# kcleal/pywfa

Hardware: AMD Instinct MI355X
Metric: pairwise alignments/sec (higher is better)
Workload: dtype int16x2 offsets (reads <= 512 bp), int32 results; 1 GPU; C2: 10000000 x 150bp pairs/GPU, 2% error, gap-affine 0/4/6/2, end-to-end, scope=score, 2-bit reads resident in HBM; pairs_per_gpu=10000000, read_length=150, parallelism=pairs sharded over 1 GPU(s), no collective

## Files before the change

pywfa_amd/csrc/host_core.hpp:

```cpp
#pragma once
#include <hip/hip_runtime.h>
#include <stdint.h>
#include <stdio.h>
#include <stdlib.h>
#include <string.h>
#include <limits.h>
#include <sched.h>
#include <string>
#include <map>
#include <unordered_map>
#include <vector>
#include <algorithm>
#include <thread>
#include <memory>
#include <atomic>

#include "wfa_hip.h"
#include "wfa_common.hpp"
#include "wfa_band.hpp"

namespace wfa { struct WfaPieceDesc; }

#pragma GCC visibility push(hidden)

extern thread_local std::string g_error;

#define WFA_COUNTER_WORDS 256
#define WFA_KNOBS(F)                                                                                              \
  F(ARENA_KB) F(BAND_DEBUG) F(BAND_SLIM) F(BAND_LDS_MAX) F(BAND_NO_WIN) F(BAND_SPLIT_MIN) F(NO_TINY_INLINE) F(BILEVEL) F(BILEVEL_WIDE_LEVELS) F(BILEVEL_PER_CU) F(BILEVEL_I32) F(BILEVEL_QCAP) F(BILEVEL_LEVELS) F(BILEVEL_LDS) F(BILEVEL_NO_1024) F(BILEVEL_HUGE_MIN) F(BILEVEL_LDS_W) F(BILEVEL_NO_SEQL) F(LANE_DYN) F(LANE_DYN_WAVES) F(BAND_LEFTOVER_WAVES_PER_CU) F(BAND_NCH) F(BAND_NO_LDS) F(BAND_NO_SPLIT) F(BAND_PB) F(PIPE_TAIL) F(LEN16) F(MAILBOX) F(MAILBOX_IDLE_US) F(TILE32)     \
  F(BAND_RECORDS) F(BAND_SPLIT_ROUNDS) F(BAND_WAVES_PER_CU) F(NO_BAND) F(NO_FAST) F(NO_SEGFULL) F(SEGFULL_PAIRS)     \
  F(SEGFULL_STAGES) F(STAGE_TIMING) F(LANE_HEUR32) F(THREADS) F(TINY_BATCH) F(WAVES_PER_CU) F(FAST_WAVES_PER_CU) F(TIMING)          \
  F(LANE_FULL) F(LANE_FULL_SPLIT) F(LANE_HEUR) F(SEG_HEUR) F(LANE_LDS_PAD_KB) F(LANE_MIN_PAIRS) F(PIPE_CHUNK) F(PIPE_THREADS) F(PACK_THREADS) F(NO_TINY_BAND) F(NO_TINY_POLL) F(UP_STREAMS) F(NO_DUAL) F(NO_WIDE) F(WIDE_ADAPT) F(WIDE_GROWS) F(WIDE_LDS_KB) F(WIDE_THREADS) F(TILE) F(TILE_T) F(TILE_WT) F(TILE_THREADS) F(TILE_PER_CU) F(NO_PIPE) F(HOST_PACK) F(GENERAL_PB) F(LANE_WAVES_PER_CU) F(LANE_REFILL_MIN) F(LANE_DEBUG) F(NO_TINY) F(PILOT_PCT) F(WIDE_ADAPT_LDS) F(LANE_NARROW_WAVES) F(PILOT_NARROW_PCT) F(CROSS_BAND) F(CROSS_TOPK_CHUNK) F(REDUCE_TIMING)
enum WfaKnob {
#define WFA_KNOB_ENUM(n) K_##n,
  WFA_KNOBS(WFA_KNOB_ENUM)
#undef WFA_KNOB_ENUM
  K_COUNT
};
struct WfaKnobs {
  int value[K_COUNT];
  bool set[K_COUNT];
  std::string fast_stages;
  void load() {
    static const char* const names[K_COUNT] = {
#define WFA_KNOB_NAME(n) "WFA_HIP_" #n,
        WFA_KNOBS(WFA_KNOB_NAME)
#undef WFA_KNOB_NAME
    };
    for (int i = 0; i < K_COUNT; ++i) {
      const char* v = getenv(names[i]);
      set[i] = v && *v;
      value[i] = set[i] ? atoi(v) : 0;
    }
    const char* fs = getenv("WFA_HIP_FAST_STAGES");
    fast_stages = (fs && *fs) ? fs : "";
  }
};

struct wfa_hip_aligner {
  int numa_state = 0;
  int numa_node = -1;
  cpu_set_t numa_cpus;
  int numa_mode = 0;
  cpu_set_t proc_cpus;
  bool proc_cpus_valid = false;
// ... 174 lines not shown
```

pywfa_amd/csrc/wfa_hip.hip:

```cpp
#include <hip/hip_runtime.h>
#include <stdint.h>
#include <stdio.h>
#include <stdlib.h>
#include <string.h>
#include <limits.h>
#include <string>
#include <map>
#include <unordered_map>
#include <vector>
#include <algorithm>
#include <chrono>
#include <thread>
#include <memory>
#include <atomic>
#include <mutex>
#include <functional>
#include <ctype.h>
#include <pthread.h>
#include <sched.h>
#include <unistd.h>
#include <sys/syscall.h>

#include "host_core.hpp"
#include "wfa_pack.hpp"
// ... 1107 lines not shown
  }
  al->err = "pilot launch failed";
  return WFA_HIP_EDEVICE;
}

static int pilot_first_width(wfa_hip_aligner* al, wfa_hip_batch* b, hipStream_t stream) {
  const unsigned rtc_failures = wfa::rtc_failure_count();
  const bool full = (b->cfg.scope == WFA_SCOPE_FULL);
  if (b->stage_pick != 0 || b->n_packed < 65536u) return WFA_HIP_OK;
  if (!wfa::seg_supported(b->dcfg, b->ncomp, false) || b->max_len > WFA_FAST_MAX_LEN || knob(al, K_NO_FAST, 0) != 0) return WFA_HIP_OK;
  if (full ? (knob(al, K_NO_SEGFULL, 0) != 0 || al->knobs.set[K_SEGFULL_STAGES]) : !al->knobs.fast_stages.empty()) return WFA_HIP_OK;
  const uint32_t np = 8192u, stride = b->n_packed / np;
  uint32_t* plist = b->d_fb_list2[0];
  uint32_t* psample = b->d_fb_list2[1];
  uint32_t* pcount = b->d_counters + 4;
  hipLaunchKernelGGL(wfa_pilot_sample_kernel, dim3((np + 255u) / 256u), dim3(256), 0, stream, b->d_list_packed, stride, np, psample);
  HIP_TRY(al, hipGetLastError());
  b->stage_pick = 128;
  for (int w = 16; w <= 64; w *= 2) {
    HIP_TRY(al, hipMemsetAsync(pcount, 0, sizeof(uint32_t), stream));
    if (wfa::launch_seg(b->dcfg, al->cu_count, knob(al, K_FAST_WAVES_PER_CU, 256), stream, b->d_words, b->d_meta, psample, nullptr, np, b->d_score, b->d_status,
                        plist, pcount, w == 16 ? 2 : (w == 32 ? 4 : 5)) != 0) return pilot_launch_failed(al, b, rtc_failures);
    uint32_t handed = 0;
    HIP_TRY(al, hipMemcpyAsync(&handed, pcount, sizeof(uint32_t), hipMemcpyDeviceToHost, stream));
    HIP_TRY(al, hipStreamSynchronize(stream));
    const uint32_t pct = (w == 16) ? (uint32_t)knob(al, K_PILOT_PCT, full ? 15 : 8) : 40u;
    if (knob(al, K_STAGE_TIMING, 0)) fprintf(stderr, "[wfa_hip] pilot: %d diagonals hand on %u of %u\n", w, handed, np);
    if (handed * 100u <= np * pct) { b->stage_pick = w; break; }
  }
  int X, OE, E;
  if (!full && b->stage_pick == 16 && wfa::seg_shape(b->dcfg, &X, &OE, &E) != WFA_SHAPE_RTC) {
    HIP_TRY(al, hipMemsetAsync(pcount, 0, sizeof(uint32_t), stream));
    if (wfa::launch_lane(wfa::seg_shape(b->dcfg, &X, &OE, &E), wfa::gcd_int(wfa::gcd_int(b->dcfg.x, b->dcfg.o1 + b->dcfg.e1), b->dcfg.e1), al->cu_count,
                         knob(al, K_LANE_WAVES_PER_CU, 48), knob(al, K_LANE_REFILL_MIN, 8), b->max_len, stream, b->d_words, b->d_meta, psample, nullptr, np,
                         b->d_score, b->d_status, plist, pcount, nullptr, 0, X, OE, E, 0, nullptr, 0, 4) != 0) return pilot_launch_failed(al, b, rtc_failures);
    uint32_t handed = 0;
    HIP_TRY(al, hipMemcpyAsync(&handed, pcount, sizeof(uint32_t), hipMemcpyDeviceToHost, stream));
    HIP_TRY(al, hipStreamSynchronize(stream));
    const uint32_t pct = (uint32_t)knob(al, K_PILOT_NARROW_PCT, 20);
    if (knob(al, K_STAGE_TIMING, 0)) fprintf(stderr, "[wfa_hip] pilot: 8 diagonals (lane form) hand on %u of %u\n", handed, np);
    b->narrow_pick = (handed * 100u <= np * pct) ? 1 : 2;
    b->narrow_permille = (int)((uint64_t)handed * 1000u / np);
  }
  HIP_TRY(al, hipMemsetAsync(pcount, 0, sizeof(uint32_t), stream));
  return WFA_HIP_OK;
}

static int pilot_band(wfa_hip_aligner* al, wfa_hip_batch* b, hipStream_t stream) {
  const unsigned rtc_failures = wfa::rtc_failure_count();
  if (b->band_pick != 0 || b->n_packed < 32768u) return WFA_HIP_OK;
  const bool two = b->ncomp == 5;
  if (b->dcfg.heuristic != WFA_HEUR_NONE || (b->ncomp != 3 && !two) || (two ? (b->max_len <= 100 || b->max_len > 2000) : (b->max_len <= 300 || b->max_len > 1200))) return WFA_HIP_OK;
  if (!wfa::band_supported(b->dcfg, b->ncomp) || knob(al, K_NO_BAND, 0) != 0 || knob(al, K_BAND_NCH, 0) != 0) return WFA_HIP_OK;
  const uint32_t np = 4096u, stride = b->n_packed / np;
  uint32_t* plist = b->d_fb_list2[0];
  uint32_t* psample = b->d_fb_list2[1];
  uint32_t* pcount = b->d_counters + 4;
  hipLaunchKernelGGL(wfa_pilot_sample_kernel, dim3((np + 255u) / 256u), dim3(256), 0, stream, b->d_list_packed, stride, np, psample);
  HIP_TRY(al, hipGetLastError());
  HIP_TRY(al, hipMemsetAsync(pcount, 0, sizeof(uint32_t), stream));
  wfa::BandArgs ba;
  memset(&ba, 0, sizeof(ba));
  ba.words = b->d_words; ba.meta = b->d_meta; ba.worklist = psample; ba.nwork = np;
  ba.score = b->d_score; ba.status = b->d_status; ba.fb_list = plist; ba.fb_count = pcount;
  fill_band_penalties(ba, b->dcfg, two);
  fill_heuristic(ba, b->dcfg);
  ba.xdrop = b->dcfg.xdrop; ba.scope = b->dcfg.scope;
// ... 946 lines not shown
  const char* stages_env = al->knobs.fast_stages.empty() ? nullptr : al->knobs.fast_stages.c_str();
  const char* stages = stages_env ? stages_env : "189";
  if (!stages_env && b->stage_pick != 0 && c.in_count == nullptr) {
    stages = (b->stage_pick == 16) ? (b->narrow_pick == 1 ? "0189" : "189") : (b->stage_pick == 32) ? "89" : "9";
  }
  int variants[6] = {-1, -1, -1, -1, -1, -1};
  int nv = 0;
  for (const char* c = stages; *c && nv < 6; ++c) {
    const int v = *c - '0';
    if (v < 0 || v > 9) continue;
    if (v <= 1) {
      if (p.shape == WFA_SHAPE_RTC && (v == 0 || !p.lane_shape_fits)) continue;
    }
    variants[nv++] = v;
  }
  if (nv == 0) variants[nv++] = 6;
  int lane_passes = 0;
  for (int pass = 0; pass < nv; ++pass) {
    uint32_t* out_list = c.out_list(b);
    uint32_t* out_count = c.next_count(b);
    StageTimer timer(al, stream);
    int lrc;
    if (variants[pass] <= 1) {
      const bool narrow = variants[pass] == 0;
      const int lane_k = lane_passes++;
      uint32_t lane_dyn = (c.in_n >= 65536u && lane_k < 2) ? (uint32_t)std::max(0, knob(al, K_LANE_DYN, 192)) : 0u;
      const int dyn_waves = narrow ? knob(al, K_LANE_NARROW_WAVES, 24) : knob(al, K_LANE_DYN_WAVES, 16);
      if (lane_dyn && c.in_count != nullptr) {
        const int64_t expect = (b->narrow_permille >= 0 && variants[0] == 0) ? (int64_t)c.in_n * b->narrow_permille / 1000 : 0;
        const int64_t per_wave = expect / std::max<int64_t>(1, (int64_t)al->cu_count * dyn_waves * 2);
        lane_dyn = (uint32_t)std::max<int64_t>(64, std::min<int64_t>(lane_dyn, per_wave));
      }
      lrc = wfa::launch_lane(p.shape, affine_gcd(b->dcfg), al->cu_count,
                             lane_dyn ? dyn_waves : knob(al, K_LANE_WAVES_PER_CU, 48), knob(al, K_LANE_REFILL_MIN, 8), b->max_len, stream, b->d_words, b->d_meta,
                             c.in_list, c.in_count, c.in_n, b->d_score, b->d_status, out_list, out_count,
                             (knob(al, K_LANE_DEBUG, 0) && al->ws) ? al->ws : nullptr, knob(al, K_LANE_LDS_PAD_KB, 0), p.sh_x, p.sh_oe, p.sh_e, knob(al, K_LANE_MIN_PAIRS, 0),
                             b->d_counters + (lane_k == 0 ? CNT_LANE_DYN0 : CNT_LANE_DYN1), lane_dyn, narrow ? 4 : 8);
      if (knob(al, K_LANE_DEBUG, 0) && al->ws) {
        unsigned long long c[10] = {0, 0, 0, 0, 0, 0, 0, 0, 0, 0};
        hipStreamSynchronize(stream); hipMemcpy(c, al->ws, sizeof(c), hipMemcpyDeviceToHost); hipMemset(al->ws, 0, sizeof(c));
        fprintf(stderr, "[wfa_hip] lane kernel: %llu wave-steps, %llu refills, %llu parked runs, %llu parked rounds, %llu probe blocks, %llu second-run rounds, "
                        "%llu hand-over blocks, %llu second runs, %llu entries, %llu entry rounds\n", c[0], c[1], c[2], c[3], c[4], c[5], c[6], c[7], c[8], c[9]);
      }
    } else {
      lrc = wfa::launch_seg(b->dcfg, al->cu_count, knob(al, K_FAST_WAVES_PER_CU, 256), stream, b->d_words, b->d_meta, c.in_list, c.in_count,
                            c.in_n, b->d_score, b->d_status, out_list, out_count, variants[pass]);
    }
    if (lrc != 0) { al->err = "fast kernel launch failed"; return WFA_HIP_EDEVICE; }
    if (timer.on) {
      uint32_t handed = 0;
      const float ms = timer.stop(out_count, &handed);
      fprintf(stderr, "[wfa_hip] stage %d (variant %d): %.3f ms, handed on %u pairs\n", pass, variants[pass], ms, handed);
    }
    c.advance(b, out_list, out_count);
  }
  return WFA_HIP_OK;
}

static int run_laneh_stage(wfa_hip_aligner* al, wfa_hip_batch* b, hipStream_t stream, const CascadePlan& p, Chain& c) {
  uint32_t* out_list = c.out_list(b);
  uint32_t* out_count = c.next_count(b);
  wfa::FastArgs fa;
  memset(&fa, 0, sizeof(fa));
  fa.words = b->d_words; fa.meta = b->d_meta; fa.worklist = c.in_list; fa.nwork_dev = c.in_count; fa.nwork = c.in_n;
  fa.score = b->d_score; fa.status = b->d_status; fa.fb_list = out_list; fa.fb_count = out_count;
  fa.g = affine_gcd(b->dcfg);
  fill_ends_free(fa, b->dcfg, true);
// ... 1071 lines not shown
```

pywfa_amd/csrc/wfa_lane.hpp:

```cpp
#pragma once
#include "wfa_rtc_compat.hpp"
#include "wfa_common.hpp"
#include "wfa_hip.h"
#ifndef __HIPCC_RTC__
#include "wfa_rtc.hpp"
#endif

namespace wfa {

typedef short lane_s2 __attribute__((ext_vector_type(2)));
typedef unsigned short lane_u2 __attribute__((ext_vector_type(2)));

#define WFA_LANE_NULL16 (-16384)
#define WFA_LANE_NULL2 0xC000C000u
#ifndef WFA_LANE_DEBUG_COUNTERS
#define WFA_LANE_DEBUG_COUNTERS 0
#endif
#ifndef WFA_LANE_REGION_MARKS
#define WFA_LANE_REGION_MARKS 0
#endif
#if WFA_LANE_REGION_MARKS
#define WFA_LANE_MARK(name) asm volatile("; WFA_MARK " name ::: "memory")
#else
#define WFA_LANE_MARK(name)
// ... 36 lines not shown
#endif
}

#ifndef WFA_LANE_WAVES_PER_EU
#define WFA_LANE_WAVES_PER_EU 0
#endif
#if WFA_LANE_WAVES_PER_EU > 0
#define WFA_LANE_OCCUPANCY __attribute__((amdgpu_waves_per_eu(WFA_LANE_WAVES_PER_EU, WFA_LANE_WAVES_PER_EU)))
#else
constexpr int lane_narrow_waves(int X, int OE, int E) {
  const int R = ((X > OE) ? X : OE) + 2 * E + 2;
  return R <= 6 ? 7 : R <= 8 ? 6 : R <= 11 ? 5 : 4;
}
#define WFA_LANE_OCCUPANCY __attribute__((amdgpu_waves_per_eu((NRP == 4) ? lane_narrow_waves(X, OE, E) : 1)))
#endif

template <int OE, int E>
struct LaneFull { static constexpr int NREC = 2 * (OE - E) + E * 17 + 1; };

template <int X, int OE, int E, bool FULL, bool HEUR = false, int LIN = 0, int NRP = 8>
__global__ void __launch_bounds__(64) WFA_LANE_OCCUPANCY
wfa_lane_kernel(const FastArgs a, const int slot_words_seq, const int refill_arg) {
  static_assert(!(FULL && HEUR), "the general form is score only");
  static_assert(NRP == 8 || (HEUR && NRP == 16) || (NRP == 4 && !FULL && !HEUR && LIN == 0),
                "the wider band exists in the general form only, the narrow one in the plain score-only form only");
  const int refill_min = refill_arg & 0xff;
  constexpr int NR = NRP, W = 2 * NR, H = NR;
  constexpr int DM = (X > OE) ? X : OE;
  constexpr int NEVER = 0x7fffffff;
  constexpr bool ENTRY = !FULL && !HEUR && LIN == 0;
  constexpr int K = ENTRY ? OE : 0, NCH = (OE + X - 1) / X;
  constexpr bool WINCH = ENTRY && NCH <= 2;
  constexpr uint32_t LNM = WINCH ? 0x3ffu : 0xffffu;
  constexpr int NREC = LaneFull<OE, E>::NREC;
  extern __shared__ uint32_t lds[];
  const int slot_words = slot_words_seq;
  const int lane = threadIdx.x;
  uint32_t nwork = __builtin_amdgcn_readfirstlane(a.nwork_dev ? *a.nwork_dev : a.nwork);
  const bool dyn = !FULL && a.dyn_next != nullptr;
  bool exhausted = !dyn;
  uint32_t begin, end;
  auto grab = [&](uint32_t& b_, uint32_t& e_) -> bool {
    uint32_t nb = 0;
    if (lane == 0) nb = atomicAdd(a.dyn_next, a.dyn_chunk);
    nb = __builtin_amdgcn_readfirstlane(nb);
    if (nb >= nwork) return false;
    b_ = nb; e_ = (uint32_t)min((unsigned long long)nwork, (unsigned long long)nb + a.dyn_chunk);
    return true;
  };
  if (dyn) {
    if (!grab(begin, end)) return;
  } else {
    const uint32_t per = __builtin_amdgcn_readfirstlane((nwork + gridDim.x - 1) / gridDim.x);
    const unsigned long long begin64 = (unsigned long long)blockIdx.x * per;
    if (begin64 >= nwork) return;
    begin = (uint32_t)begin64;
    end = (uint32_t)min((unsigned long long)nwork, begin64 + per);
  }

  uint32_t pid0, pw0, ln0, pid1, pw1, ln1;
  __shared__ short wch[(WINCH && NCH == 2) ? 128 : 1];
  auto window_chain = [&](uint32_t wb, uint32_t pw, uint32_t ln) -> uint32_t {
    WFA_LANE_MARK("entry_begin");
    WFA_LANE_COUNT(8);
    const int pl = (int)(ln & 0xffffu), tl = (int)(ln >> 16);
    const int nwp = (pl + 15) >> 4, ntot = nwp + ((tl + 15) >> 4), ak = tl - pl, L = min(pl, tl);
    const bool elig = (unsigned long long)wb + lane < end &&
                      !(ln == 0xffffffffu || ntot + 1 > slot_words_seq || ak < 1 - 2 * H || ak > 2 * H - 1);
    bool act = elig;
    const uint32_t* pp = a.words + pw;
    int ch[NCH];
#pragma unroll
    for (int c = 0; c < NCH; ++c) ch[c] = WFA_LANE_NULL16;
    int ci = 0;
    const int imax = slot_words_seq >> 1;
    int base = 0;
#pragma nounroll
    for (int i = 0; i < imax && __any(act); i += 2) {
      WFA_LANE_MARK("entryround_begin");
      WFA_LANE_COUNT(9);
      uint32_t x0 = 0u, x1 = 0u;
      if (act && base < L) x0 = pp[0] ^ pp[nwp];
      if (act && base + 16 < L) x1 = pp[1] ^ pp[nwp + 1];
      unsigned long long d = (unsigned long long)((x0 | (x0 >> 1)) & 0x55555555u) | ((unsigned long long)((x1 | (x1 >> 1)) & 0x55555555u) << 32);
#pragma unroll
      for (int c = 0; c < NCH; ++c) {
        const int pos = d ? base + ((int)__builtin_ctzll(d) >> 1) : 0x7fff;
        const bool hit = act && pos < L;
#pragma unroll
        for (int k = 0; k < NCH; ++k) ch[k] = (hit && ci == k) ? pos : ch[k];
        ci += hit ? 1 : 0;
        act = act && ci < NCH;
        d &= d - 1ull;
      }
      const bool endc = act && base + 32 >= L;
#pragma unroll
      for (int k = 0; k < NCH; ++k) ch[k] = (endc && ci == k) ? L : ch[k];
      act = act && !endc;
      pp += 2; base += 32;
      WFA_LANE_MARK("entryround_end");
    }
    if constexpr (NCH == 2) wch[64 + lane] = (short)ch[1];
    WFA_LANE_MARK("entry_end");
    const uint32_t c0 = (uint32_t)ch[0];
    return elig ? (ln | ((c0 & 0x3fu) << 10) | ((c0 >> 6) << 26)) : ln;
  };
  auto load_window = [&](uint32_t wb, uint32_t& pid, uint32_t& pw, uint32_t& ln) {
    const unsigned long long idx = (unsigned long long)wb + lane;
    pid = 0u; pw = 0u; ln = 0u;
    if (idx < end) {
      pid = a.worklist ? a.worklist[a.work_begin + idx] : (uint32_t)(a.work_begin + idx);
      const WfaPairMeta m = a.meta[pid];
      pw = m.p_woff;
      ln = (m.plen > WFA_FAST_MAX_LEN || m.tlen > WFA_FAST_MAX_LEN) ? 0xffffffffu : ((uint32_t)m.plen | ((uint32_t)m.tlen << 16));
    }
  };
  uint32_t wbase = begin, next_i = begin;
  uint32_t wneed = 2u;
  bool wmeta = false;
  if constexpr (!WINCH) {
    load_window(wbase, pid0, pw0, ln0);
    load_window(wbase + 64u, pid1, pw1, ln1);
  } else {
    pid0 = pw0 = ln0 = pid1 = pw1 = ln1 = 0u;
  }

  const int pbase = (4 + lane * slot_words) * 16;
  uint32_t cur[NR], lim[NR], Mh[DM][NR], Ih[E][NR], Dh[E][NR];
  uint32_t thr[HEUR ? NR : 1];
#pragma unroll
  for (int r = 0; r < NR; ++r) {
    cur[r] = WFA_LANE_NULL2; lim[r] = WFA_LANE_NULL2;
    if (HEUR) thr[r] = 0x3fff3fffu;
#pragma unroll
    for (int d = 0; d < DM; ++d) Mh[d][r] = WFA_LANE_NULL2;
#pragma unroll
    for (int d = 0; d < E; ++d) { Ih[d][r] = WFA_LANE_NULL2; Dh[d][r] = WFA_LANE_NULL2; }
  }
  int kb0 = pbase, tb = pbase;
  int jt = 0;
  uint32_t tend = 0xffffu;
  int s0 = 0, deadline = NEVER;
  uint32_t my_lb2 = 0, my_tl2 = 0;
  int steps_wait = 0, my_dinit = 0;
  bool edge_live = false;
  uint32_t mypid = 0;
  unsigned long long idle = ~0ull;
  int gstep = 0;
  uint32_t myslot = 0;
  uint2* const wave_codes = FULL ? a.codes + (unsigned long long)blockIdx.x * (unsigned long long)a.codes_cap * 64ull : nullptr;
  bool codes_full = false;
  __shared__ uint32_t rejq[128];
  int nrej = 0;
  auto rej_flush = [&]() {
    if (nrej == 0) return;
    uint32_t slot = 0;
    if (lane == 0) slot = atomicAdd(a.fb_count, (uint32_t)nrej);
    slot = __builtin_amdgcn_readfirstlane(slot);
    if (lane < nrej) a.fb_list[slot + lane] = rejq[lane];
    if (lane + 64 < nrej) a.fb_list[slot + 64 + lane] = rejq[64 + lane];
    nrej = 0;
  };

  while (true) {
    WFA_LANE_MARK("looptop_begin");
    const int nidle = __builtin_popcountll(idle);
    if (!exhausted && next_i >= end && (nidle >= refill_min || idle == ~0ull)) {
      if (grab(begin, end)) {
        wbase = begin; next_i = begin;
        if constexpr (WINCH) { wneed = 2u; wmeta = false; }
        else { load_window(wbase, pid0, pw0, ln0); load_window(wbase + 64u, pid1, pw1, ln1); }
      } else exhausted = true;
    }
    if (next_i < end && (nidle >= refill_min || idle == ~0ull)) {
      WFA_LANE_MARK("refill_begin");
      WFA_LANE_COUNT(1);
      if constexpr (WINCH) {
#pragma nounroll
        for (; wneed; --wneed) {
          const uint32_t wb = wneed == 2u ? wbase : wbase + 64u;
          if (!wmeta) load_window(wb, pid1, pw1, ln1);
          wmeta = false;
          ln1 = window_chain(wb, pw1, ln1);
          if (wneed == 2u) {
            pid0 = pid1; pw0 = pw1; ln0 = ln1;
            if constexpr (NCH == 2) wch[lane] = wch[64 + lane];
          }
        }
      }
      const bool is_idle = __builtin_amdgcn_inverse_ballot_w64(idle);
      const uint32_t rank = __builtin_amdgcn_mbcnt_hi((uint32_t)(idle >> 32), __builtin_amdgcn_mbcnt_lo((uint32_t)idle, 0u));
      const uint32_t navail = end - next_i;
      const bool take = is_idle && rank < navail;
      const uint32_t src = next_i + rank - wbase;
      const int sl = (int)(src & 63u);
      const uint32_t a_pid = __shfl(pid0, sl, 64), a_pw = __shfl(pw0, sl, 64), a_ln = __shfl(ln0, sl, 64);
      const uint32_t b_pid = __shfl(pid1, sl, 64), b_pw = __shfl(pw1, sl, 64), b_ln = __shfl(ln1, sl, 64);
      const bool hi_w = src >= 64u;
      const uint32_t n_pid = hi_w ? b_pid : a_pid, n_pw = hi_w ? b_pw : a_pw, n_ln = hi_w ? b_ln : a_ln;
      const int pl = (int)(n_ln & LNM), tl = (int)((n_ln >> 16) & LNM);
      const int nwp = (pl + 15) >> 4, ntot = nwp + ((tl + 15) >> 4);
      const int ak = tl - pl;
      const int pbf_ = (HEUR && a.ef) ? a.pbf : 0, tbf_ = (HEUR && a.ef) ? a.tbf : 0;
      const int dlo = min(-pbf_, ak), dhi = max(tbf_, ak);
      const bool bad = n_ln == 0xffffffffu || ntot + 1 > slot_words_seq ||
                       (HEUR ? (dhi - dlo > 2 * H - 3) : (ak < 1 - 2 * H || ak > 2 * H - 1));
      const unsigned long long tmask = __ballot(take);
      {
        unsigned long long lm = __ballot(take && !bad);
        while (lm) {
          const int L = __builtin_ctzll(lm);
          lm &= lm - 1ull;
          const uint32_t pw = __builtin_amdgcn_readlane(n_pw, L);
          const int nt = __builtin_amdgcn_readlane(ntot, L);
          if (lane < nt) __builtin_amdgcn_global_load_lds(a.words + pw + lane, &lds[4 + L * slot_words], 4, 0, 0);
        }
      }
      if (take) {
        const int c = bad ? 0 : (HEUR ? ((dlo + dhi + 1) >> 1) : ((ak + 1) >> 1));
        const int k0 = c - H;
        mypid = n_pid; s0 = gstep - K;
        if (FULL) myslot = next_i + rank;
        kb0 = pbase - k0; tb = pbase + nwp * 16;
        jt = bad ? 0 : ak - k0;
        tend = bad ? 0xffffu : (uint32_t)tl;
        deadline = bad ? gstep - 1
                       : HEUR ? gstep + 4 * (pl + tl) + 64
                       : s0 + min(2 * (OE - E) + E * (2 * c + 2 * H - ak), 2 * (OE - E) + E * (2 * H + 2 - 2 * c + ak))
                               - (FULL ? 1 : 0);
        const int j0 = -k0;
        const uint32_t lb2 = ((uint32_t)(pl + k0) & 0xffffu) | ((uint32_t)(pl + k0 + 1) << 16);
        const uint32_t tl2 = (uint32_t)tl | ((uint32_t)tl << 16);
        const int j0r = bad ? -1 : (j0 >> 1);
        const uint32_t c0 = (j0 & 1) ? ((uint32_t)WFA_LANE_NULL16 & 0xffffu) : (WFA_LANE_NULL2 & 0xffff0000u);
        if (HEUR) { my_lb2 = lb2; my_tl2 = tl2; steps_wait = a.steps_between; my_dinit = max(pl, tl); }
#pragma unroll
        for (int r = 0; r < NR; ++r) {
          lim[r] = bad ? WFA_LANE_NULL2 : pk_min(tl2, pk_add(lb2, (uint32_t)(2 * r) * 0x00010001u));
          cur[r] = (!ENTRY && j0r == r) ? c0 : WFA_LANE_NULL2;
          if (HEUR) {
            uint32_t c2 = 0, t2 = 0;
#pragma unroll
            for (int q = 0; q < 2; ++q) {
              const int k = k0 + 2 * r + q;
              int w0v = (k == 0) ? 0 : WFA_LANE_NULL16;
              if (a.ef && k >= -pbf_ && k <= tbf_) w0v = max(k, 0);
              int th = (k == ak) ? tl : 0x3fff;
              if (a.ef) th = min(max(tl, pl + k - a.pef), max(pl + k, tl - a.tef));
              if (bad) { w0v = WFA_LANE_NULL16; th = 0x3fff; }
              th = max(0, min(th, 0x3fff));
              c2 |= ((uint32_t)w0v & 0xffffu) << (16 * q);
              t2 |= ((uint32_t)th & 0xffffu) << (16 * q);
            }
            cur[r] = c2; thr[r] = t2;
          }
#pragma unroll
          for (int d = 0; d < DM; ++d) Mh[d][r] = WFA_LANE_NULL2;
#pragma unroll
          for (int d = 0; d < E; ++d) { Ih[d][r] = WFA_LANE_NULL2; Dh[d][r] = WFA_LANE_NULL2; }
        }
      }
      const uint32_t ntake = min((uint32_t)nidle, navail);
      next_i += ntake;
      idle &= ~tmask;
      if constexpr (!WINCH) {
        __builtin_amdgcn_s_waitcnt(0x0F70);
        asm volatile("" ::: "memory");
      }
      if constexpr (ENTRY) {
        const bool go = take && !bad;
        if (__any(go)) {
          int ch[NCH];
          int fin_i = -1;
          if constexpr (WINCH) {
            ch[0] = (int)(((n_ln >> 10) & 0x3fu) | (((n_ln >> 26) & 0xfu) << 6));
            if constexpr (NCH == 2) ch[1] = (int)wch[src];
#pragma unroll
            for (int i = 0; i < NCH; ++i) fin_i = (ak == 0 && ch[i] == tl) ? i : fin_i;
          } else {
            WFA_LANE_MARK("entry_begin");
            WFA_LANE_COUNT(8);
#pragma unroll
            for (int i = 0; i < NCH; ++i) ch[i] = WFA_LANE_NULL16;
            const int etb = go ? tb : pbase;
            int ci = 0, ex = 0, lf = go ? min(pl, tl) : 0;
            bool act = go;
            do {
              WFA_LANE_MARK("entryround_begin");
              WFA_LANE_COUNT(9);
              const int v = ex + pbase, h = ex + etb;
              const uint32_t pa = ((uint32_t)v >> 2) & ~3u, ta = ((uint32_t)h >> 2) & ~3u;
              const uint32_t* pp = reinterpret_cast<const uint32_t*>(reinterpret_cast<const char*>(lds) + pa);
              const uint32_t* tp = reinterpret_cast<const uint32_t*>(reinterpret_cast<const char*>(lds) + ta);
              const uint32_t p0 = pp[0], p1 = pp[1], p2 = pp[2], t0 = tp[0], t1 = tp[1], t2 = tp[2];
              const uint32_t xl = __builtin_amdgcn_alignbit(p1, p0, (uint32_t)v << 1) ^ __builtin_amdgcn_alignbit(t1, t0, (uint32_t)h << 1);
              const uint32_t xh = __builtin_amdgcn_alignbit(p2, p1, (uint32_t)v << 1) ^ __builtin_amdgcn_alignbit(t2, t1, (uint32_t)h << 1);
              const uint32_t fb = min(lane_ffbl(xl), lane_ffbl(xh) | 32u);
              const int m = min((int)(fb >> 1), min(32, lf));
              ex += m; lf -= m;
              const bool stop = act && !((m == 32) && (lf > 0));
#pragma unroll
              for (int i = 0; i < NCH; ++i) ch[i] = (stop && ci == i) ? ex : ch[i];
              fin_i = (stop && ak == 0 && ex == tl) ? ci : fin_i;
              ci += stop ? 1 : 0;
              const bool on = stop && ci < NCH && lf > 0;
              act = stop ? on : act;
              ex += on ? 1 : 0; lf -= on ? 1 : 0;
              WFA_LANE_MARK("entryround_end");
            } while (__any(act));
            WFA_LANE_MARK("entry_end");
          }
          const bool fin = go && fin_i >= 0;
          if (fin) {
            a.score[mypid] = -__mul24(fin_i * X, a.g);
            a.status[mypid] = 0;
          }
          idle |= __ballot(fin);
          if (go) {
            auto place = [&](uint32_t (&dst)[NR], int slot, int val) {
              const int rr = fin ? -1 : (slot >> 1);
              const uint32_t w = (slot & 1) ? (((uint32_t)WFA_LANE_NULL16 & 0xffffu) | ((uint32_t)val << 16))
                                            : ((WFA_LANE_NULL2 & 0xffff0000u) | ((uint32_t)val & 0xffffu));
#pragma unroll
              for (int r = 0; r < NR; ++r) dst[r] = (rr == r) ? w : WFA_LANE_NULL2;
            };
            const int j0 = H - ((ak + 1) >> 1);
#pragma unroll
            for (int d = 0; d < DM; ++d) {
              const int sc = K - 1 - d;
              if (sc >= 0 && sc % X == 0) place(Mh[d], j0, ch[sc / X]);
            }
            place(Ih[0], j0 + 1, ch[0] + 1);
            place(Dh[0], j0 - 1, ch[0]);
            uint32_t mm[NR];
            if (K % X == 0) place(mm, j0, ch[NCH - 1] + 1);
#pragma unroll
            for (int r = 0; r < NR; ++r) {
              const uint32_t gap = pk_max(Ih[0][r], Dh[0][r]);
              cur[r] = pk_clamp((K % X == 0) ? pk_max(gap, mm[r]) : gap, lim[r]);
              if (fin) lim[r] = WFA_LANE_NULL2;
            }
            if (fin) { deadline = NEVER; jt = 0; tend = 0xffffu; }
          }
        }
      }
      if constexpr (WINCH) {
        __builtin_amdgcn_s_waitcnt(0x0F70);
        asm volatile("" ::: "memory");
      }
      if (next_i - wbase >= 64u) {
        pid0 = pid1; pw0 = pw1; ln0 = ln1; wbase += 64u;
        if constexpr (WINCH) {
          if constexpr (NCH == 2) wch[lane] = wch[64 + lane];
          wneed = 1u; wmeta = true;
        }
        load_window(wbase + 64u, pid1, pw1, ln1);
      }
      WFA_LANE_MARK("refill_end");
    } else if (idle == ~0ull && exhausted) {
      rej_flush();
      break;
    }

    int hot_j = -1, hot_x = 0, hot_left = 0;
#pragma unroll
    for (int r = 0; r < NR; ++r) {
      const uint32_t ua = pk_min(cur[r], pk_add(pk_sub(lim[r], cur[r]), 0xffffffffu));
      if (__any((ua & 0x80008000u) != 0x80008000u)) {
        WFA_LANE_MARK("probe_begin");
        WFA_LANE_COUNT(4);
        int off[2], left[2], x[2];
        bool valid[2], more[2];
#pragma unroll
        for (int q = 0; q < 2; ++q) {
          off[q] = q ? ((int)cur[r] >> 16) : (int)(short)(cur[r] & 0xffffu);
          const int lj = q ? ((int)lim[r] >> 16) : (int)(short)(lim[r] & 0xffffu);
          valid[q] = off[q] >= 0;
          left[q] = valid[q] ? lj - off[q] : 0;
        }
#pragma unroll
        for (int q = 0; q < 2; ++q) {
          const int j = 2 * r + q;
          x[q] = max(off[q], 0);
          const int v = x[q] + kb0 - j, h = x[q] + tb;
          const uint32_t pa = ((uint32_t)v >> 2) & ~3u, ta = ((uint32_t)h >> 2) & ~3u;
          const uint32_t* pp = reinterpret_cast<const uint32_t*>(reinterpret_cast<const char*>(lds) + pa);
          const uint32_t* tp = reinterpret_cast<const uint32_t*>(reinterpret_cast<const char*>(lds) + ta);
          const uint32_t p0 = pp[0], p1 = pp[1], t0 = tp[0], t1 = tp[1];
          const uint32_t xl = __builtin_amdgcn_alignbit(p1, p0, (uint32_t)v << 1) ^ __builtin_amdgcn_alignbit(t1, t0, (uint32_t)h << 1);
          const int m = min((int)(lane_ffbl(xl) >> 1), min(16, left[q]));
          x[q] += m; left[q] -= m;
// ... 88 lines not shown
      unsigned long long blimit = 0ull;
      if constexpr (HEUR) blimit = __ballot(a.max_steps != NEVER && __mul24(gstep - s0 + 1, a.g) >= a.max_steps) & active & ~bfin;
      const unsigned long long brej = __ballot(gstep > deadline || (HEUR && edge_live) || (FULL && codes_full)) & active & ~blimit;
      const unsigned long long bd = bfin | brej | blimit;
      if (bd) {
        WFA_LANE_MARK("bd_begin");
        WFA_LANE_COUNT(6);
        const unsigned long long ba = bfin & ~brej;
        if (__builtin_amdgcn_inverse_ballot_w64(ba)) {
          a.score[mypid] = -__mul24(gstep - s0, a.g);
          a.status[mypid] = 0;
          if (FULL) a.end_state[myslot] = make_int4((int)(blockIdx.x * (unsigned)a.codes_cap + (unsigned)gstep), lane | (jt << 8), gstep - s0, 1);
        }
        if (HEUR && __builtin_amdgcn_inverse_ballot_w64(blimit)) {
          a.score[mypid] = -a.max_steps;
          a.status[mypid] = WFA_STATUS_MAX_STEPS_REACHED;
        }
        if (brej) {
          if (__builtin_amdgcn_inverse_ballot_w64(brej)) {
            rejq[nrej + (int)__builtin_amdgcn_mbcnt_hi((uint32_t)(brej >> 32), __builtin_amdgcn_mbcnt_lo((uint32_t)brej, 0u))] = mypid;
            a.status[mypid] = WFA_INTERNAL_FALLBACK;
            if (FULL) a.end_state[myslot] = make_int4(0, 0, 0, 0);
          }
          nrej += __builtin_popcountll(brej);
          if (nrej >= 64) rej_flush();
        }
        if (__builtin_amdgcn_inverse_ballot_w64(bd)) {
#pragma unroll
          for (int r = 0; r < NR; ++r) { cur[r] = WFA_LANE_NULL2; lim[r] = WFA_LANE_NULL2; if (HEUR) thr[r] = 0x3fff3fffu; }
          deadline = NEVER; jt = 0; tend = 0xffffu; edge_live = false;
        }
        idle |= bd;
        WFA_LANE_MARK("bd_end");
        if (idle == ~0ull && next_i >= end && exhausted) { rej_flush(); break; }
      }
    }

    if constexpr (HEUR) {
      if (a.heur == 1) {
        auto mask16 = [&](const uint32_t (&x)[NR]) -> uint32_t {
          uint32_t lo16 = 0, hi16 = 0;
#pragma unroll
          for (int r = 0; r < NR; ++r) {
            const lane_u2 t = __builtin_bit_cast(lane_u2, x[r]) >> (unsigned short)15;
            const uint32_t w = (1u << (2 * (r & 7))) | (1u << (2 * (r & 7) + 17));
            if (r < 8) lo16 = __builtin_amdgcn_udot2(t, __builtin_bit_cast(lane_u2, w), lo16, false);
            else hi16 = __builtin_amdgcn_udot2(t, __builtin_bit_cast(lane_u2, w), hi16, false);
          }
          return ~(lo16 | (hi16 << 16)) & (NR == 16 ? 0xffffffffu : 0xffffu);
        };
        const uint32_t live = mask16(cur);
        if (live != 0u) --steps_wait;
        const int lo = (int)lane_ffbl(live), hi = 31 - (int)__builtin_clz(live | 1u);
        const bool consider = live != 0u && steps_wait <= 0 && (hi - lo + 1) >= a.min_wf_len && !__builtin_amdgcn_inverse_ballot_w64(idle);
        if (__any(consider)) {
          uint32_t d2[NR];
          uint32_t dm = 0x3fff3fffu;
#pragma unroll
          for (int r = 0; r < NR; ++r) {
            const uint32_t dl = pk_max(my_tl2, pk_add(my_lb2, (uint32_t)(2 * r) * 0x00010001u));
            const uint32_t dv = pk_sub(dl, cur[r]);
            const uint32_t dead = __builtin_bit_cast(uint32_t, __builtin_bit_cast(lane_s2, cur[r]) >> (short)15);
            d2[r] = (dv & ~dead) | (0x3fff3fffu & dead);
            dm = pk_min(dm, d2[r]);
          }
          const int dmin = min(my_dinit, min((int)(dm & 0xffffu), (int)(dm >> 16)));
          const uint32_t lim2 = (uint32_t)min(dmin + min(a.max_dist_thr, 0x3ffe), 0x3ffe) * 0x00010001u;
// ... 85 lines not shown
      }
    }
    ++gstep;
  }
  if (WFA_LANE_DEBUG_COUNTERS && !FULL && a.hist) { if (lane == 0) atomicAdd(reinterpret_cast<unsigned long long*>(a.hist), (unsigned long long)gstep); }
}

#ifndef __HIPCC_RTC__
#define WFA_LANE_DECL(i, x, oe, e) \
  int launch_lane_s##i(unsigned grid, size_t smem, hipStream_t stream, const FastArgs& a, int slot_words, int refill_min, bool full, int heur, int nrp);
WFA_LANE_DECL(0, 2, 4, 1) WFA_LANE_DECL(1, 2, 3, 1) WFA_LANE_DECL(2, 4, 7, 1) WFA_LANE_DECL(3, 3, 5, 1)
WFA_LANE_DECL(4, 6, 8, 3) WFA_LANE_DECL(5, 5, 3, 3) WFA_LANE_DECL(6, 1, 2, 1)
#undef WFA_LANE_DECL

template <int X, int OE, int E>
inline int launch_lane_shape(unsigned grid, size_t smem, hipStream_t stream, const FastArgs& a, int slot_words, int refill_min, bool full, int heur, int nrp) {
  if (nrp == 4 && (full || heur)) return -1;
  if (nrp == 4) hipLaunchKernelGGL((wfa_lane_kernel<X, OE, E, false, false, 0, 4>), dim3(grid), dim3(64), smem, stream, a, slot_words, refill_min);
  else if (heur == 2) hipLaunchKernelGGL((wfa_lane_kernel<X, OE, E, false, true, 0, 16>), dim3(grid), dim3(64), smem, stream, a, slot_words, refill_min);
  else if (heur) hipLaunchKernelGGL((wfa_lane_kernel<X, OE, E, false, true>), dim3(grid), dim3(64), smem, stream, a, slot_words, refill_min);
  else if (full) hipLaunchKernelGGL((wfa_lane_kernel<X, OE, E, true>), dim3(grid), dim3(64), smem, stream, a, slot_words, refill_min);
  else hipLaunchKernelGGL((wfa_lane_kernel<X, OE, E, false>), dim3(grid), dim3(64), smem, stream, a, slot_words, refill_min);
  return hipGetLastError() == hipSuccess ? 0 : -1;
}

inline bool lane_heur_config(const WfaDevConfig& c, int ncomp) {
  return ncomp == 3 && c.match == 0 && c.wildcard < 0 && (c.heuristic == 0 || c.heuristic == 1);
}

inline int lane_slot_words(int max_len) {
  const int w = 2 * ((max_len + 15) >> 4) + 1;
  return w | 1;
}

inline int lane_full_records(int OE, int E) { return 2 * (OE - E) + E * 17 + 1; }
inline void lane_full_geometry(uint32_t nwork, int cu_count, int per_cu, int min_pairs, int OE, int E, long long* grid_out, int* cap_out) {
  if (min_pairs <= 0) min_pairs = 256;
  long long grid = (long long)cu_count * per_cu;
  const long long max_grid = ((long long)nwork + min_pairs - 1) / std::max(min_pairs, 64);
  if (grid > max_grid) grid = max_grid;
  if (grid < 1) grid = 1;
  const long long per = ((long long)nwork + grid - 1) / grid;
  const int nrec = lane_full_records(OE, E);
  *grid_out = grid;
  *cap_out = (int)(per * nrec / 32 + 2 * nrec + 8);
}

#define WFA_LANE_RUN_SLOT 32

inline int launch_lane_args(int shape_idx, int OE, int E, int cu_count, int per_cu, int refill_min, int max_len, hipStream_t stream, FastArgs a, bool full, int lds_pad_kb = 0, int min_pairs = 0, int heur = 0, int X = 0, int nrp = 8);

inline int launch_lane(int shape_idx, int g, int cu_count, int per_cu, int refill_min, int max_len, hipStream_t stream, const uint32_t* words,
                       const WfaPairMeta* meta, const uint32_t* worklist, const uint32_t* nwork_dev, uint32_t nwork,
                       int32_t* score, int32_t* status, uint32_t* fb_list, uint32_t* fb_count, int32_t* debug_counters = nullptr, int lds_pad_kb = 0,
                       int X = 0, int OE = 0, int E = 0, int min_pairs = 0, uint32_t* dyn_next = nullptr, uint32_t dyn_chunk = 0, int nrp = 8) {
  FastArgs a = FastArgs();
  a.dyn_next = dyn_chunk ? dyn_next : nullptr; a.dyn_chunk = dyn_chunk;
  a.words = words; a.meta = meta; a.worklist = worklist; a.nwork_dev = nwork_dev; a.nwork = nwork;
  a.score = score; a.status = status; a.fb_list = fb_list; a.fb_count = fb_count;
  a.g = g;
  a.hist = debug_counters; a.hist_stride = 0; a.end_state = nullptr; a.work_begin = 0;
  a.ef = a.pbf = a.pef = a.tbf = a.tef = 0; a.heur = 0; a.min_wf_len = a.max_dist_thr = a.steps_between = 0; a.max_steps = INT_MAX;
  return launch_lane_args(shape_idx, OE, E, cu_count, per_cu, refill_min, max_len, stream, a, false, lds_pad_kb, min_pairs, 0, X, nrp);
}

inline int launch_lane_args(int shape_idx, int OE, int E, int cu_count, int per_cu, int refill_min, int max_len, hipStream_t stream, FastArgs a, bool full, int lds_pad_kb, int min_pairs, int heur, int X, int nrp) {
// ... 35 lines not shown
```

Baseline: 4.271 billion alignments/s.

## Finish low-mismatch equal-length pairs during window prescan and compact survivors

During the windowed entry-chain prescan, pairs with equal lengths now also get a full Hamming-mismatch count. Those whose mismatches stay within a bound derived from the gap-affine costs get their score written immediately and never occupy a wavefront lane. The remaining pairs in each 64-entry window are compacted with ds_permute, and the refill logic now tracks variable-size windows (wn0/wp0/wn1) instead of fixed 64-pair strides. This removes per-lane WFA work for near-identical pairs, at the cost of extra popcounts, a permute, and more complex window bookkeeping. It is enabled by default through a new knob bit packed into refill_min.

```diff
diff --git a/pywfa_amd/csrc/host_core.hpp b/pywfa_amd/csrc/host_core.hpp
--- a/pywfa_amd/csrc/host_core.hpp
+++ b/pywfa_amd/csrc/host_core.hpp
@@ -30,7 +30,7 @@
   F(ARENA_KB) F(BAND_DEBUG) F(BAND_SLIM) F(BAND_LDS_MAX) F(BAND_NO_WIN) F(BAND_SPLIT_MIN) F(NO_TINY_INLINE) F(BILEVEL) F(BILEVEL_WIDE_LEVELS) F(BILEVEL_PER_CU) F(BILEVEL_I32) F(BILEVEL_QCAP) F(BILEVEL_LEVELS) F(BILEVEL_LDS) F(BILEVEL_NO_1024) F(BILEVEL_HUGE_MIN) F(BILEVEL_LDS_W) F(BILEVEL_NO_SEQL) F(LANE_DYN) F(LANE_DYN_WAVES) F(BAND_LEFTOVER_WAVES_PER_CU) F(BAND_NCH) F(BAND_NO_LDS) F(BAND_NO_SPLIT) F(BAND_PB) F(PIPE_TAIL) F(LEN16) F(MAILBOX) F(MAILBOX_IDLE_US) F(TILE32)     \
   F(BAND_RECORDS) F(BAND_SPLIT_ROUNDS) F(BAND_WAVES_PER_CU) F(NO_BAND) F(NO_FAST) F(NO_SEGFULL) F(SEGFULL_PAIRS)     \
   F(SEGFULL_STAGES) F(STAGE_TIMING) F(LANE_HEUR32) F(THREADS) F(TINY_BATCH) F(WAVES_PER_CU) F(FAST_WAVES_PER_CU) F(TIMING)          \
-  F(LANE_FULL) F(LANE_FULL_SPLIT) F(LANE_HEUR) F(SEG_HEUR) F(LANE_LDS_PAD_KB) F(LANE_MIN_PAIRS) F(PIPE_CHUNK) F(PIPE_THREADS) F(PACK_THREADS) F(NO_TINY_BAND) F(NO_TINY_POLL) F(UP_STREAMS) F(NO_DUAL) F(NO_WIDE) F(WIDE_ADAPT) F(WIDE_GROWS) F(WIDE_LDS_KB) F(WIDE_THREADS) F(TILE) F(TILE_T) F(TILE_WT) F(TILE_THREADS) F(TILE_PER_CU) F(NO_PIPE) F(HOST_PACK) F(GENERAL_PB) F(LANE_WAVES_PER_CU) F(LANE_REFILL_MIN) F(LANE_DEBUG) F(NO_TINY) F(PILOT_PCT) F(WIDE_ADAPT_LDS) F(LANE_NARROW_WAVES) F(PILOT_NARROW_PCT) F(CROSS_BAND) F(CROSS_TOPK_CHUNK) F(REDUCE_TIMING)
+  F(LANE_FULL) F(LANE_FULL_SPLIT) F(LANE_HEUR) F(SEG_HEUR) F(LANE_LDS_PAD_KB) F(LANE_MIN_PAIRS) F(PIPE_CHUNK) F(PIPE_THREADS) F(PACK_THREADS) F(NO_TINY_BAND) F(NO_TINY_POLL) F(UP_STREAMS) F(NO_DUAL) F(NO_WIDE) F(WIDE_ADAPT) F(WIDE_GROWS) F(WIDE_LDS_KB) F(WIDE_THREADS) F(TILE) F(TILE_T) F(TILE_WT) F(TILE_THREADS) F(TILE_PER_CU) F(NO_PIPE) F(HOST_PACK) F(GENERAL_PB) F(LANE_WAVES_PER_CU) F(LANE_REFILL_MIN) F(LANE_WINFIN) F(LANE_DEBUG) F(NO_TINY) F(PILOT_PCT) F(WIDE_ADAPT_LDS) F(LANE_NARROW_WAVES) F(PILOT_NARROW_PCT) F(CROSS_BAND) F(CROSS_TOPK_CHUNK) F(REDUCE_TIMING)
 enum WfaKnob {
 #define WFA_KNOB_ENUM(n) K_##n,
   WFA_KNOBS(WFA_KNOB_ENUM)
diff --git a/pywfa_amd/csrc/wfa_hip.hip b/pywfa_amd/csrc/wfa_hip.hip
--- a/pywfa_amd/csrc/wfa_hip.hip
+++ b/pywfa_amd/csrc/wfa_hip.hip
@@ -1163,7 +1163,7 @@
   if (!full && b->stage_pick == 16 && wfa::seg_shape(b->dcfg, &X, &OE, &E) != WFA_SHAPE_RTC) {
     HIP_TRY(al, hipMemsetAsync(pcount, 0, sizeof(uint32_t), stream));
     if (wfa::launch_lane(wfa::seg_shape(b->dcfg, &X, &OE, &E), wfa::gcd_int(wfa::gcd_int(b->dcfg.x, b->dcfg.o1 + b->dcfg.e1), b->dcfg.e1), al->cu_count,
-                         knob(al, K_LANE_WAVES_PER_CU, 48), knob(al, K_LANE_REFILL_MIN, 8), b->max_len, stream, b->d_words, b->d_meta, psample, nullptr, np,
+                         knob(al, K_LANE_WAVES_PER_CU, 48), wfa::lane_refill_arg(knob(al, K_LANE_REFILL_MIN, 8), knob(al, K_LANE_WINFIN, 1) != 0), b->max_len, stream, b->d_words, b->d_meta, psample, nullptr, np,
                          b->d_score, b->d_status, plist, pcount, nullptr, 0, X, OE, E, 0, nullptr, 0, 4) != 0) return pilot_launch_failed(al, b, rtc_failures);
     uint32_t handed = 0;
     HIP_TRY(al, hipMemcpyAsync(&handed, pcount, sizeof(uint32_t), hipMemcpyDeviceToHost, stream));
@@ -2176,7 +2176,8 @@
         lane_dyn = (uint32_t)std::max<int64_t>(64, std::min<int64_t>(lane_dyn, per_wave));
       }
       lrc = wfa::launch_lane(p.shape, affine_gcd(b->dcfg), al->cu_count,
-                             lane_dyn ? dyn_waves : knob(al, K_LANE_WAVES_PER_CU, 48), knob(al, K_LANE_REFILL_MIN, 8), b->max_len, stream, b->d_words, b->d_meta,
+                             lane_dyn ? dyn_waves : knob(al, K_LANE_WAVES_PER_CU, 48),
+                             wfa::lane_refill_arg(knob(al, K_LANE_REFILL_MIN, 8), knob(al, K_LANE_WINFIN, 1) != 0), b->max_len, stream, b->d_words, b->d_meta,
                              c.in_list, c.in_count, c.in_n, b->d_score, b->d_status, out_list, out_count,
                              (knob(al, K_LANE_DEBUG, 0) && al->ws) ? al->ws : nullptr, knob(al, K_LANE_LDS_PAD_KB, 0), p.sh_x, p.sh_oe, p.sh_e, knob(al, K_LANE_MIN_PAIRS, 0),
                              b->d_counters + (lane_k == 0 ? CNT_LANE_DYN0 : CNT_LANE_DYN1), lane_dyn, narrow ? 4 : 8);
diff --git a/pywfa_amd/csrc/wfa_lane.hpp b/pywfa_amd/csrc/wfa_lane.hpp
--- a/pywfa_amd/csrc/wfa_lane.hpp
+++ b/pywfa_amd/csrc/wfa_lane.hpp
@@ -92,6 +92,9 @@
   constexpr int K = ENTRY ? OE : 0, NCH = (OE + X - 1) / X;
   constexpr bool WINCH = ENTRY && NCH <= 2;
   constexpr uint32_t LNM = WINCH ? 0x3ffu : 0xffffu;
+  constexpr int MH = (2 * OE) / X;
+  static_assert(NCH - 1 <= MH && MH * X <= 2 * OE, "the chain's own end cells lie within the Hamming bound");
+  const int mh = (refill_arg & 0x100) ? MH : NCH - 1;
   constexpr int NREC = LaneFull<OE, E>::NREC;
   extern __shared__ uint32_t lds[];
   const int slot_words = slot_words_seq;
@@ -120,14 +123,16 @@
 
   uint32_t pid0, pw0, ln0, pid1, pw1, ln1;
   __shared__ short wch[(WINCH && NCH == 2) ? 128 : 1];
-  auto window_chain = [&](uint32_t wb, uint32_t pw, uint32_t ln) -> uint32_t {
+  auto window_chain = [&](uint32_t wb, uint32_t& pid, uint32_t& pw, uint32_t& ln) -> uint32_t {
     WFA_LANE_MARK("entry_begin");
     WFA_LANE_COUNT(8);
     const int pl = (int)(ln & 0xffffu), tl = (int)(ln >> 16);
     const int nwp = (pl + 15) >> 4, ntot = nwp + ((tl + 15) >> 4), ak = tl - pl, L = min(pl, tl);
-    const bool elig = (unsigned long long)wb + lane < end &&
-                      !(ln == 0xffffffffu || ntot + 1 > slot_words_seq || ak < 1 - 2 * H || ak > 2 * H - 1);
+    const bool inw = (unsigned long long)wb + lane < end;
+    const bool elig = inw && !(ln == 0xffffffffu || ntot + 1 > slot_words_seq || ak < 1 - 2 * H || ak > 2 * H - 1);
     bool act = elig;
+    bool hact = elig && ak == 0, hend = false;
+    int hm = 0;
     const uint32_t* pp = a.words + pw;
     int ch[NCH];
 #pragma unroll
@@ -136,34 +141,59 @@
     const int imax = slot_words_seq >> 1;
     int base = 0;
 #pragma nounroll
-    for (int i = 0; i < imax && __any(act); i += 2) {
+    for (int i = 0; i < imax && __any(act || hact); i += 2) {
       WFA_LANE_MARK("entryround_begin");
       WFA_LANE_COUNT(9);
       uint32_t x0 = 0u, x1 = 0u;
-      if (act && base < L) x0 = pp[0] ^ pp[nwp];
-      if (act && base + 16 < L) x1 = pp[1] ^ pp[nwp + 1];
-      unsigned long long d = (unsigned long long)((x0 | (x0 >> 1)) & 0x55555555u) | ((unsigned long long)((x1 | (x1 >> 1)) & 0x55555555u) << 32);
+      const bool on = act || hact;
+      if (on && base < L) x0 = pp[0] ^ pp[nwp];
+      if (on && base + 16 < L) x1 = pp[1] ^ pp[nwp + 1];
+      const int nb = L - base;
+      const uint32_t k0 = nb >= 16 ? 0x55555555u : nb > 0 ? (0x55555555u >> (32 - 2 * nb)) : 0u;
+      const uint32_t k1 = nb >= 32 ? 0x55555555u : nb > 16 ? (0x55555555u >> (64 - 2 * nb)) : 0u;
+      unsigned long long d = (unsigned long long)((x0 | (x0 >> 1)) & k0) | ((unsigned long long)((x1 | (x1 >> 1)) & k1) << 32);
+      hm += hact ? (int)__builtin_popcountll(d) : 0;
 #pragma unroll
       for (int c = 0; c < NCH; ++c) {
-        const int pos = d ? base + ((int)__builtin_ctzll(d) >> 1) : 0x7fff;
-        const bool hit = act && pos < L;
+        const int pos = base + ((int)__builtin_ctzll(d | (1ull << 63)) >> 1);
+        const bool hit = act && d != 0ull;
 #pragma unroll
         for (int k = 0; k < NCH; ++k) ch[k] = (hit && ci == k) ? pos : ch[k];
         ci += hit ? 1 : 0;
         act = act && ci < NCH;
         d &= d - 1ull;
       }
-      const bool endc = act && base + 32 >= L;
+      const bool last = base + 32 >= L;
+      const bool endc = act && last;
 #pragma unroll
       for (int k = 0; k < NCH; ++k) ch[k] = (endc && ci == k) ? L : ch[k];
       act = act && !endc;
+      hend = hend || (hact && last);
+      hact = hact && !last && hm <= mh;
       pp += 2; base += 32;
       WFA_LANE_MARK("entryround_end");
     }
-    if constexpr (NCH == 2) wch[64 + lane] = (short)ch[1];
+    const bool fin = hend && hm <= mh;
+    if (fin) {
+      a.score[pid] = -__mul24(hm * X, a.g);
+      a.status[pid] = 0;
+    }
+    const uint32_t c0 = (uint32_t)ch[0];
+    uint32_t lnc = elig ? (ln | ((c0 & 0x3fu) << 10) | ((c0 >> 6) << 26)) : ln;
+    const bool keep = inw && !fin;
+    const unsigned long long km = __ballot(keep);
+    int dst = lane;
+    if (__ballot(fin)) {
+      const int rk = (int)__builtin_amdgcn_mbcnt_hi((uint32_t)(km >> 32), __builtin_amdgcn_mbcnt_lo((uint32_t)km, 0u));
+      dst = keep ? rk : (int)__builtin_popcountll(km) + lane - rk;
+      pid = (uint32_t)__builtin_amdgcn_ds_permute(dst << 2, (int)pid);
+      pw = (uint32_t)__builtin_amdgcn_ds_permute(dst << 2, (int)pw);
+      lnc = (uint32_t)__builtin_amdgcn_ds_permute(dst << 2, (int)lnc);
+    }
+    if constexpr (NCH == 2) wch[64 + dst] = (short)ch[1];
+    ln = lnc;
     WFA_LANE_MARK("entry_end");
-    const uint32_t c0 = (uint32_t)ch[0];
-    return elig ? (ln | ((c0 & 0x3fu) << 10) | ((c0 >> 6) << 26)) : ln;
+    return (uint32_t)__builtin_popcountll(km);
   };
   auto load_window = [&](uint32_t wb, uint32_t& pid, uint32_t& pw, uint32_t& ln) {
     const unsigned long long idx = (unsigned long long)wb + lane;
@@ -176,8 +206,12 @@
     }
   };
   uint32_t wbase = begin, next_i = begin;
-  uint32_t wneed = 2u;
+  uint32_t wn0 = 0u, wp0 = 0u, wn1 = 0u, wnext = begin;
   bool wmeta = false;
+  auto slice_done = [&]() -> bool {
+    if constexpr (WINCH) return wp0 >= wn0 && wn1 == 0u && wnext >= end;
+    else return next_i >= end;
+  };
   if constexpr (!WINCH) {
     load_window(wbase, pid0, pw0, ln0);
     load_window(wbase + 64u, pid1, pw1, ln1);
@@ -225,38 +259,39 @@
   while (true) {
     WFA_LANE_MARK("looptop_begin");
     const int nidle = __builtin_popcountll(idle);
-    if (!exhausted && next_i >= end && (nidle >= refill_min || idle == ~0ull)) {
+    if (!exhausted && slice_done() && (nidle >= refill_min || idle == ~0ull)) {
       if (grab(begin, end)) {
         wbase = begin; next_i = begin;
-        if constexpr (WINCH) { wneed = 2u; wmeta = false; }
+        if constexpr (WINCH) { wn0 = wp0 = wn1 = 0u; wnext = begin; wmeta = false; }
         else { load_window(wbase, pid0, pw0, ln0); load_window(wbase + 64u, pid1, pw1, ln1); }
       } else exhausted = true;
     }
-    if (next_i < end && (nidle >= refill_min || idle == ~0ull)) {
+    if (!slice_done() && (nidle >= refill_min || idle == ~0ull)) {
       WFA_LANE_MARK("refill_begin");
       WFA_LANE_COUNT(1);
       if constexpr (WINCH) {
 #pragma nounroll
-        for (; wneed; --wneed) {
-          const uint32_t wb = wneed == 2u ? wbase : wbase + 64u;
-          if (!wmeta) load_window(wb, pid1, pw1, ln1);
+        while (wn1 == 0u && wnext < end) {
+          if (!wmeta) load_window(wnext, pid1, pw1, ln1);
           wmeta = false;
-          ln1 = window_chain(wb, pw1, ln1);
-          if (wneed == 2u) {
+          wn1 = window_chain(wnext, pid1, pw1, ln1);
+          wnext = (end - wnext > 64u) ? wnext + 64u : end;
+          if (wp0 >= wn0) {
             pid0 = pid1; pw0 = pw1; ln0 = ln1;
             if constexpr (NCH == 2) wch[lane] = wch[64 + lane];
+            wn0 = wn1; wp0 = 0u; wn1 = 0u;
           }
         }
       }
       const bool is_idle = __builtin_amdgcn_inverse_ballot_w64(idle);
       const uint32_t rank = __builtin_amdgcn_mbcnt_hi((uint32_t)(idle >> 32), __builtin_amdgcn_mbcnt_lo((uint32_t)idle, 0u));
-      const uint32_t navail = end - next_i;
+      const uint32_t navail = WINCH ? (wn0 - wp0) + wn1 : end - next_i;
       const bool take = is_idle && rank < navail;
-      const uint32_t src = next_i + rank - wbase;
-      const int sl = (int)(src & 63u);
+      const uint32_t src = WINCH ? wp0 + rank : next_i + rank - wbase;
+      const bool hi_w = src >= (WINCH ? wn0 : 64u);
+      const int sl = (int)((WINCH ? (hi_w ? src - wn0 : src) : src) & 63u);
       const uint32_t a_pid = __shfl(pid0, sl, 64), a_pw = __shfl(pw0, sl, 64), a_ln = __shfl(ln0, sl, 64);
       const uint32_t b_pid = __shfl(pid1, sl, 64), b_pw = __shfl(pw1, sl, 64), b_ln = __shfl(ln1, sl, 64);
-      const bool hi_w = src >= 64u;
       const uint32_t n_pid = hi_w ? b_pid : a_pid, n_pw = hi_w ? b_pw : a_pw, n_ln = hi_w ? b_ln : a_ln;
       const int pl = (int)(n_ln & LNM), tl = (int)((n_ln >> 16) & LNM);
       const int nwp = (pl + 15) >> 4, ntot = nwp + ((tl + 15) >> 4);
@@ -321,7 +356,7 @@
         }
       }
       const uint32_t ntake = min((uint32_t)nidle, navail);
-      next_i += ntake;
+      if constexpr (WINCH) wp0 += ntake; else next_i += ntake;
       idle &= ~tmask;
       if constexpr (!WINCH) {
         __builtin_amdgcn_s_waitcnt(0x0F70);
@@ -331,15 +366,14 @@
         const bool go = take && !bad;
         if (__any(go)) {
           int ch[NCH];
-          int fin_i = -1;
+          bool fin = false;
           if constexpr (WINCH) {
             ch[0] = (int)(((n_ln >> 10) & 0x3fu) | (((n_ln >> 26) & 0xfu) << 6));
-            if constexpr (NCH == 2) ch[1] = (int)wch[src];
-#pragma unroll
-            for (int i = 0; i < NCH; ++i) fin_i = (ak == 0 && ch[i] == tl) ? i : fin_i;
+            if constexpr (NCH == 2) ch[1] = (int)wch[(hi_w ? 64 : 0) + sl];
           } else {
             WFA_LANE_MARK("entry_begin");
             WFA_LANE_COUNT(8);
+            int fin_i = -1;
 #pragma unroll
             for (int i = 0; i < NCH; ++i) ch[i] = WFA_LANE_NULL16;
             const int etb = go ? tb : pbase;
@@ -369,16 +403,16 @@
               WFA_LANE_MARK("entryround_end");
             } while (__any(act));
             WFA_LANE_MARK("entry_end");
+            fin = go && fin_i >= 0;
+            if (fin) {
+              a.score[mypid] = -__mul24(fin_i * X, a.g);
+              a.status[mypid] = 0;
+            }
+            idle |= __ballot(fin);
           }
-          const bool fin = go && fin_i >= 0;
-          if (fin) {
-            a.score[mypid] = -__mul24(fin_i * X, a.g);
-            a.status[mypid] = 0;
-          }
-          idle |= __ballot(fin);
           if (go) {
             auto place = [&](uint32_t (&dst)[NR], int slot, int val) {
-              const int rr = fin ? -1 : (slot >> 1);
+              const int rr = (!WINCH && fin) ? -1 : (slot >> 1);
               const uint32_t w = (slot & 1) ? (((uint32_t)WFA_LANE_NULL16 & 0xffffu) | ((uint32_t)val << 16))
                                             : ((WFA_LANE_NULL2 & 0xffff0000u) | ((uint32_t)val & 0xffffu));
 #pragma unroll
@@ -398,9 +432,9 @@
             for (int r = 0; r < NR; ++r) {
               const uint32_t gap = pk_max(Ih[0][r], Dh[0][r]);
               cur[r] = pk_clamp((K % X == 0) ? pk_max(gap, mm[r]) : gap, lim[r]);
-              if (fin) lim[r] = WFA_LANE_NULL2;
+              if constexpr (!WINCH) { if (fin) lim[r] = WFA_LANE_NULL2; }
             }
-            if (fin) { deadline = NEVER; jt = 0; tend = 0xffffu; }
+            if constexpr (!WINCH) { if (fin) { deadline = NEVER; jt = 0; tend = 0xffffu; } }
           }
         }
       }
@@ -408,15 +442,19 @@
         __builtin_amdgcn_s_waitcnt(0x0F70);
         asm volatile("" ::: "memory");
       }
-      if (next_i - wbase >= 64u) {
+      if constexpr (WINCH) {
+        if (wp0 >= wn0) {
+          pid0 = pid1; pw0 = pw1; ln0 = ln1;
+          if constexpr (NCH == 2) wch[lane] = wch[64 + lane];
+          wp0 -= wn0; wn0 = wn1; wn1 = 0u;
+          if (wnext < end) { load_window(wnext, pid1, pw1, ln1); wmeta = true; }
+        }
+      } else if (next_i - wbase >= 64u) {
         pid0 = pid1; pw0 = pw1; ln0 = ln1; wbase += 64u;
-        if constexpr (WINCH) {
-          if constexpr (NCH == 2) wch[lane] = wch[64 + lane];
-          wneed = 1u; wmeta = true;
-        }
         load_window(wbase + 64u, pid1, pw1, ln1);
       }
       WFA_LANE_MARK("refill_end");
+      if (WINCH && ntake == 0u && idle == ~0ull) continue;
     } else if (idle == ~0ull && exhausted) {
       rej_flush();
       break;
@@ -571,7 +609,7 @@
         }
         idle |= bd;
         WFA_LANE_MARK("bd_end");
-        if (idle == ~0ull && next_i >= end && exhausted) { rej_flush(); break; }
+        if (idle == ~0ull && slice_done() && exhausted) { rej_flush(); break; }
       }
     }
 
@@ -723,6 +761,8 @@
   const int w = 2 * ((max_len + 15) >> 4) + 1;
   return w | 1;
 }
+
+inline int lane_refill_arg(int refill_min, bool winfin) { return (refill_min & 0xff) | (winfin ? 0x100 : 0); }
 
 inline int lane_full_records(int OE, int E) { return 2 * (OE - E) + E * 17 + 1; }
 inline void lane_full_geometry(uint32_t nwork, int cu_count, int per_cu, int min_pairs, int OE, int E, long long* grid_out, int* cap_out) {
```

Result: faster. 4.386 billion alignments/s (median of 6 runs) (+2.7%).
